# fperezgamonal/flownet2-tf

Hardware: AMD Instinct MI355X
Metric: forward pairs/sec at 512x384 (FlowNet2) (higher is better)
Workload: dtype f16x2 (split fp16 hi+lo operands, 3 fp16 MFMAs per product, fp32 accumulate); 1 GPU; FlowNet2 forward, batch=4 synthetic 512x384 pairs per GPU, seeded synthetic weights; pairs_per_gpu=4, parallelism=dp1 (no collective)

## Files before the change

### flownet2-tf_amd/csrc/conv.hip

```cpp
#include "conv_common.h"
#include <cstdlib>

namespace fn2 {

template <typename T, typename OutT, int TC, int WC, int WP>
__global__ void __launch_bounds__(256) conv_igemm_kernel(const ConvArgs p) {
  constexpr int CH = 16 / (int)sizeof(T);
  constexpr int BC = WC * TC * 16;
  constexpr int BP = WP * 64;
  constexpr int NT = 256;
  static_assert(WC * WP == 4, "4 waves per block");
  constexpr int NPR = BP / 64;
  constexpr int NWR = (BC * 4 + NT - 1) / NT;
  constexpr int WSWZ_BIT = (TC == 4) ? 5 : (TC == 2) ? 4 : 3;
  __shared__ uint4 lds[2][(BC + BP) * 4];

  const int tid = threadIdx.x, lane = tid & 63, wave = tid >> 6;
  const int wc = wave / WP, wp = wave % WP;
  const int cid = tid & 3;

  int pad_y = p.pad, pad_x = p.pad, oy_off = 0, ox_off = 0, osc = 1;
  const T* wgt = reinterpret_cast<const T*>(p.wgt);
  const int phase = blockIdx.z / p.splitk, split = blockIdx.z - phase * p.splitk;
  if (p.deconv) {
// ... 528 lines not shown
      if (oy >= 0 && oy < H && ox >= 0 && ox < W) {
        const bool inner = ey >= E && ey < E + TY && ex >= E && ex < E + TX;
        float2* po = reinterpret_cast<float2*>(pf + (((long)n * H + oy) * W + ox) * 2);
        if (ring && (oy == 0 || oy == H - 1 || ox == 0 || ox == W - 1)) {
          const float2 v = *po;
          a0 = v.x; a1 = v.y;
        } else {
          a0 = b0; a1 = b1;
#pragma unroll
          for (int ky = 0; ky < NT; ++ky)
#pragma unroll
            for (int kx = 0; kx < NT; ++kx) {
              const float2 v = sm[((ey + ky) * RW + ex + kx) * NTAP + ky * NT + kx];
              a0 += v.x; a1 += v.y;
            }
          if (inner) *po = make_float2(a0, a1);
        }
      }
      spf[e] = make_float2(a0, a1);
    }
    if constexpr (UP) {
      __syncthreads();
      const float ub0 = up_bias ? up_bias[0] : 0.f, ub1 = up_bias ? up_bias[1] : 0.f;
      for (int o = tid; o < 4 * TY * TX; o += 256) {
        const int uy = o / (2 * TX), ux = o - uy * (2 * TX);
        const int oy = 2 * ty * TY + uy, ox = 2 * tx * TX + ux;
        if (oy >= 2 * H || ox >= 2 * W) continue;
        const int a = uy & 1, b = ux & 1, y = uy >> 1, x = ux >> 1;
        float r0 = ub0, r1 = ub1;
#pragma unroll
        for (int tty = 0; tty < 2; ++tty) {
          const int iy = y - 1 + a + tty, ky = 3 - a - 2 * tty;
          const int gy = ty * TY + iy;
          if (gy < 0 || gy >= H) continue;
#pragma unroll
          for (int ttx = 0; ttx < 2; ++ttx) {
            const int ix = x - 1 + b + ttx, kx = 3 - b - 2 * ttx;
            const int gx = tx * TX + ix;
            if (gx < 0 || gx >= W) continue;
            const float2 v = spf[(iy + E) * EW + ix + E];
            const float* ww = sw + (ky * 4 + kx) * 4;
            r0 += v.x * ww[0] + v.y * ww[1];
            r1 += v.x * ww[2] + v.y * ww[3];
          }
        }
        OutT* po = up + (((size_t)n * 2 * H + oy) * 2 * W + ox) * up_cs + up_c0;
        if constexpr (is_x2<OutT>::value) {
          const size_t addr = reinterpret_cast<size_t>(po);
          _Float16* g = reinterpret_cast<_Float16*>(addr & ~size_t(31));
          const int j = (int)((addr & 31) >> 2);
          typedef __attribute__((ext_vector_type(2))) _Float16 h2;
          const _Float16 h0 = (_Float16)r0, h1 = (_Float16)r1;
          *reinterpret_cast<h2*>(g + j) = h2{h0, h1};
          *reinterpret_cast<h2*>(g + 8 + j) = h2{(_Float16)(r0 - (float)h0), (_Float16)(r1 - (float)h1)};
        } else {
          store_elem<OutT>(po, r0);
          store_elem<OutT>(po + 1, r1);
        }
      }
    }
    __syncthreads();
  }
}

__global__ void __launch_bounds__(256) head_ring_kernel(const x2_t* __restrict__ in, int in_cs, int in_c0, int cin_groups,
                                                        const float* __restrict__ wc, const float* __restrict__ bc,
                                                        float* __restrict__ pf, int N, int H, int W) {
  const int lane = threadIdx.x & 63;
  const long wave = ((long)blockIdx.x * blockDim.x + threadIdx.x) >> 6;
  const long nwaves = ((long)gridDim.x * blockDim.x) >> 6;
  const int ring = 2 * W + 2 * (H - 2);
  const int nitems = 25 * cin_groups;
  const size_t case_stride = (size_t)nitems * 8 * 2;
  for (long m = wave; m < (long)N * ring; m += nwaves) {
    const int n = (int)(m / ring), r = (int)(m - (long)n * ring);
    int y, x;
    if (r < W) { y = 0; x = r; }
    else if (r < 2 * W) { y = H - 1; x = r - W; }
    else { const int q = r - 2 * W; y = 1 + (q >> 1); x = (q & 1) ? W - 1 : 0; }
    const int cy = y == 0 ? 0 : (y == H - 1 ? 2 : 1), cx = x == 0 ? 0 : (x == W - 1 ? 2 : 1);
    const int cs = 3 * cy + cx;
    const float* w = wc + (size_t)cs * case_stride;
// ... 672 lines not shown
  a.h5_tiles = (int)blocks;
  long total = blocks;
  if (ring && ring_w != nullptr) {
    FN2_REQUIRE(ring_b != nullptr, "flow_head5: ring_w without ring_b");
    a.h5_wc = ring_w; a.h5_bc = ring_b; a.h5_groups = (x->c + 7) / 8;
    FN2_REQUIRE(x->c0 + a.h5_groups * 8 <= x->cs, "flow_head5: the last 8-channel group reaches past the buffer");
    total += cdiv((long)x->n * (2 * x->w + 2 * (x->h - 2)), 16);
  }
  {
    const char* e = getenv("FN2_H5_STRIP");
    if ((a.ksteps == 3 || a.ksteps == 6) && !(e && atoi(e) == 0) && !(a.dbg & 10)) {
      const int nstrip = cdiv(x->w, 60);
      const char* eb = getenv("FN2_H5_BLOCKS");
      const int target = eb ? atoi(eb) : 256;
      const int segs = std::max(1, std::min(x->h, target / std::max(1, x->n * nstrip)));
      const int rows = cdiv(x->h, segs);
      a.h5_tx = nstrip; a.h5_ty = cdiv(x->h, rows); a.h5_rows = rows;
      return launch_head5_strip(a, x->n * a.h5_ty * a.h5_tx, (hipStream_t)stream);
    }
  }
  return launch_head5(a, (int)total, (hipStream_t)stream);
}

int fn2_flow_head_ring(const fn2_tensor* x, const float* wc, const float* bc, float* pf, void* stream) {
  int rc = check_view(x, "flow_head_ring input");
  if (rc) return rc;
  FN2_REQUIRE(wc && bc && pf, "flow_head_ring: null pointer");
  FN2_REQUIRE(x->dtype == FN2_F16X2 && x->cs % 8 == 0 && x->c0 % 8 == 0, "flow_head_ring: split-fp16 input, 8-aligned view");
  FN2_REQUIRE(x->h >= 3 && x->w >= 3, "flow_head_ring: h, w >= 3");
  const int groups = (x->c + 7) / 8;
  FN2_REQUIRE(x->c0 + groups * 8 <= x->cs, "flow_head_ring: the last 8-channel group reaches past the buffer");
  const long ring = (long)x->n * (2 * x->w + 2 * (x->h - 2));
  hipLaunchKernelGGL(head_ring_kernel, dim3(grid_for(ring * 64, 256)), dim3(256), 0, (hipStream_t)stream, (const x2_t*)x->data,
                     x->cs, x->c0, groups, wc, bc, pf, x->n, x->h, x->w);
  FN2_CHECK_LAUNCH("flow_head_ring");
  return FN2_OK;
}

int fn2_upsample_flow(const float* in, const float* w, const float* bias, const fn2_tensor* out, int n, int h, int wd,
                      void* stream) {
  FN2_REQUIRE(in && w, "upsample_flow: null pointer");
  int rc = check_view(out, "upsample_flow output");
  if (rc) return rc;
  FN2_REQUIRE(out->c == 2 && out->n == n && out->h == 2 * h && out->w == 2 * wd,
              "upsample_flow: output view must be [n, 2h, 2w, 2]");
  const long total = (long)n * 4 * h * wd;
// ... 58 lines not shown
```

### flownet2-tf_amd/csrc/conv2.hip

```cpp
#include "conv_common.h"

#include <type_traits>
#include <algorithm>
#include <utility>

#ifndef FN2_X2_ORDER
#define FN2_X2_ORDER 0
#endif
#ifndef FN2_CONV_ABLATE
#define FN2_CONV_ABLATE 0
#endif
#ifndef FN2_SETPRIO
#define FN2_SETPRIO 1
#endif

namespace fn2 {

typedef __attribute__((address_space(3))) void* lptr_t;

constexpr unsigned kOobOffset = 0x80000000u;

typedef int v4i_t __attribute__((ext_vector_type(4)));
typedef unsigned u32x4_t __attribute__((ext_vector_type(4)));

// ... 65 lines not shown
    a1 += __shfl_xor(a1, off, 64);
  }
  if (lane == 0)
    *reinterpret_cast<float2*>(pf + (((size_t)n * H + y) * W + x) * 2) = make_float2(a0 + p.h5_bc[2 * cs], a1 + p.h5_bc[2 * cs + 1]);
}

__device__ __forceinline__ void h5_ring_block(const ConvArgs& p, int rb) {
  const int wave = threadIdx.x >> 6;
  const long total = (long)p.N * (2 * p.OW + 2 * (p.OH - 2));
  for (int k = 0; k < 4; ++k) {
    const long m = (long)rb * 16 + wave * 4 + k;
    if (m >= total) return;
    h5_ring_pixel(p, m);
  }
}

__device__ __forceinline__ float* h5_t(uint4* a, uint4* b, int half, int w) {
  const int byte = w * 4;
  return byte < half ? reinterpret_cast<float*>(reinterpret_cast<char*>(a) + byte)
                     : reinterpret_cast<float*>(reinterpret_cast<char*>(b) + (byte - half));
}

template <typename T, typename OutT, int WC, int WP, int TCN = 2, int TPN = 2, int STAGES = 2, int KG = 1, bool M16 = false,
          bool WREG = false, bool SLAB = false, bool HEAD5 = false, bool FEED = false>
__global__ void __launch_bounds__(256 * KG + (FEED ? 256 : 0)) conv_igemm2_kernel(const ConvArgs p) {
#if defined(__HIP_DEVICE_COMPILE__)
  constexpr int CH = 16 / (int)sizeof(T);
  constexpr int ESZ = (int)sizeof(T);
  constexpr int BC = WC * TCN * 32, BP = WP * TPN * 32;
  static_assert(WC * WP == 4, "4 waves per block");
  constexpr int NWI = BC / 32;
  constexpr int NPI = BP / 32;
  static_assert(!WREG || (is_x2<T>::value && TCN == 1 && KG == 1 && (STAGES == 2 || STAGES == 3) && !M16),
                "WREG: split fp16, one cout tile per wave, two-stage loop or 3-slot ring");
  constexpr int BOFF = WREG ? 0 : BC;
  constexpr int kWTileBytes = (32 * TPN * (TCN * 32 + 4) + 32 * TPN) * 4;
  constexpr int kPoolHalfRows = (STAGES * BP * 128 / 2 > 2 * kWTileBytes ? STAGES * BP * 128 / 2 : 2 * kWTileBytes) / 128 + 1;
  constexpr int ROWS = WREG ? kPoolHalfRows : BC + BP;
  static_assert(KG == 1 || STAGES == 2, "K groups run the two-stage loop");
  constexpr bool kDeep = STAGES > 3;
  __shared__ uint4 lds0_all[(kDeep ? STAGES : WREG ? 2 : KG) * ROWS * 8];
  __shared__ uint4 lds1_all[(kDeep || WREG) ? 1 : KG * ROWS * 8];
  __shared__ uint4 lds2_own[(STAGES == 3 && !WREG) ? ROWS * 8 : 1];

  if constexpr (HEAD5) {
    if ((int)blockIdx.x >= p.h5_tiles) {
      h5_ring_block(p, (int)blockIdx.x - p.h5_tiles);
      return;
    }
  }
  if constexpr (WREG && SLAB && is_x2<T>::value) {
    if (p.fh_M > 0 && (int)blockIdx.z >= p.fh_z0) {
      if (FEED && threadIdx.x >= 256) return;
      float* part = reinterpret_cast<float*>(lds0_all);
      const long e = (((long)blockIdx.z - p.fh_z0) * gridDim.y + blockIdx.y) * gridDim.x + blockIdx.x;
      const long total = (long)(gridDim.z - p.fh_z0) * gridDim.y * gridDim.x;
      for (long m = e; m < p.fh_M; m += total)
        fh_pixel(reinterpret_cast<const x2_t*>(p.in), p.H, p.W, p.in_cs, p.in_c0, p.fh_groups, p.fh_w, p.fh_w + p.fh_w1,
                 p.fh_bias, p.fh_scale, p.fh_out + (size_t)m * p.fh_out_cs + p.fh_out_c0, m, part);
      return;
    }
  }
  const int tid = threadIdx.x, lane = tid & 63;
  const int wave_all = __builtin_amdgcn_readfirstlane(tid >> 6);
  const int grp = KG > 1 ? wave_all >> 2 : 0;
  static_assert(!FEED || (WREG && STAGES == 3 && KG == 1), "FEED: the WREG ring");
  const bool feeder = FEED && wave_all >= 4;
  const int wave = (KG > 1 || FEED) ? wave_all & 3 : wave_all;
  uint4* const lds0 = lds0_all + grp * (ROWS * 8);
  uint4* const lds1 = WREG ? lds0_all + BP * 8 : kDeep ? lds0_all + ROWS * 8 : lds1_all + grp * (ROWS * 8);
  uint4* const lds2 = WREG ? lds0_all + 2 * BP * 8 : lds2_own;
  uint4* const ep1 = (kDeep || WREG) ? lds0_all + ROWS * 8 : lds1_all;
  const int wc = wave / WP, wp = wave % WP;

  int pad_y = p.pad, pad_x = p.pad, oy_off = 0, ox_off = 0, osc = 1;
  const T* wgt = reinterpret_cast<const T*>(p.wgt);
  const int phase = blockIdx.z / p.splitk, split = blockIdx.z - phase * p.splitk;
  const unsigned wrow_bytes = (unsigned)p.ksteps * 128u;
  if (p.deconv) {
    const int a = phase >> 1, b = phase & 1;
    pad_y = a ? p.ph_pad1 : p.ph_pad0; pad_x = b ? p.ph_pad1 : p.ph_pad0; oy_off = a; ox_off = b; osc = 2;
    wgt += (size_t)phase * p.cout_pad * (wrow_bytes / ESZ);
  }
  const int khi = p.deconv ? p.kh_ph[phase >> 1] : p.KH, kwi = p.deconv ? p.kw_ph[phase & 1] : p.KW;
  const int nst_all = (p.cin_chunks >> 3) * khi * kwi;
  const int kt0 = split * p.kper + grp;
  const int kt1 = (FN2_CONV_ABLATE && (p.dbg & 1048576)) ? kt0 : min(nst_all, split * p.kper + p.kper);
  int bx = blockIdx.x, by = blockIdx.y;
  if (!(p.dbg & 4)) {
    const int NT = HEAD5 ? p.h5_tiles : gridDim.x * gridDim.y, L = blockIdx.x + gridDim.x * blockIdx.y;
    const int xcd = L & 7, chunk = NT >> 3, rem = NT & 7;
    const int Lp = xcd * chunk + min(xcd, rem) + (L >> 3);
    if (p.wmajor) {
      by = Lp / (int)gridDim.x;
      bx = Lp - by * (int)gridDim.x;
    } else {
      bx = Lp / (int)gridDim.y;
      by = Lp - bx * (int)gridDim.y;
    }
  }
  const int m0 = bx * BP;
  const int c0 = by * BC;

  const v4i_t rsrc_w = make_rsrc(wgt, (int)(p.cout_pad * wrow_bytes));
  const v4i_t rsrc_x = make_rsrc(p.in, p.in_bytes);

  const int lrow = lane >> 3, lphys = lane & 7;
  unsigned woff[NWI];
#pragma unroll
  for (int j = 0; j < NWI; ++j) {
    const int row = wave * (BC / 4) + j * 8 + lrow;
    woff[j] = (unsigned)(c0 + row) * wrow_bytes + (unsigned)((lphys ^ ((row >> 1) & 7)) * 16);
  }
  int roff[NPI];
  unsigned vmask[NPI];
#pragma unroll
  for (int j = 0; j < NPI; ++j) {
    const int row = wave * (BP / 4) + j * 8 + lrow;
    const int m = m0 + row;
    bool v = m < p.M;
    const int mm = v ? m : 0;
    int n = mm / (p.OH * p.OW);
    const int rem = mm - n * (p.OH * p.OW);
    int oy = rem / p.OW, ox = rem - oy * p.OW;
    if constexpr (HEAD5) {
      static_assert(BP == 256, "HEAD5: 8 x 32 positions per block");
      const int tx = bx % p.h5_tx, tyn = bx / p.h5_tx;
      n = tyn / p.h5_ty;
      oy = (tyn - n * p.h5_ty) * 4 - 2 + (row >> 5);
      ox = tx * 28 - 2 + (row & 31);
      v = true;
    }
    const int iy0 = oy * p.stride - pad_y, ix0 = ox * p.stride - pad_x;
    roff[j] = (((n * p.H + iy0) * p.W + ix0) * p.in_cs + p.in_c0) * ESZ + (lphys ^ ((row >> 1) & 7)) * 16;
    unsigned mk = 0;
    if (v) {
      for (int k = 0; k < p.KH; ++k) mk |= (unsigned)(iy0 + k >= 0 && iy0 + k < p.H) << k;
      for (int k = 0; k < p.KW; ++k) mk |= (unsigned)(ix0 + k >= 0 && ix0 + k < p.W) << (8 + k);
    }
    vmask[j] = mk;
  }
  const int spt = p.cin_chunks >> 3;
  const int ntap = khi * kwi;
  const bool tap_outer = FN2_CONV_ABLATE && (p.dbg & 16);
  int sc = tap_outer ? kt0 % spt : kt0 / ntap;
  int tap = tap_outer ? kt0 / spt : kt0 - sc * ntap;
  int ky = tap / kwi, kx = tap - ky * kwi;
  int wstage = kt0;

  auto issue_piece = [&](auto piece_c, uint4* lds) {
    constexpr int i = decltype(piece_c)::value;
    if constexpr (i < NWI) {
      if constexpr (!WREG) {
// ... 356 lines not shown
            *reinterpret_cast<float4*>(h5_t(lds0_all, lds1_all, ROWS * 128, pos * TS + cb + 4 * q)) =
                make_float4(acc[tc][tp][4 * q] * p.out_scale, acc[tc][tp][4 * q + 1] * p.out_scale,
                            acc[tc][tp][4 * q + 2] * p.out_scale, acc[tc][tp][4 * q + 3] * p.out_scale);
      }
    __syncthreads();
    if (p.dbg & 8) return;
    const int tx = bx % p.h5_tx, tyn = bx / p.h5_tx;
    const int n = tyn / p.h5_ty, ty = tyn - n * p.h5_ty;
    float* pf = reinterpret_cast<float*>(p.out);
    if (tid < 224) {
      const int o = tid & 1, px = tid >> 1;
      const int py = px / 28, pxx = px - py * 28;
      const int oy = ty * 4 + py, ox = tx * 28 + pxx;
      if (oy < p.OH && ox < p.OW && !(p.h5_ring && (oy == 0 || oy == p.OH - 1 || ox == 0 || ox == p.OW - 1))) {
        float a = p.bias ? p.bias[o] : 0.f;
#pragma unroll
        for (int uy = 0; uy < 5; ++uy)
#pragma unroll
          for (int ux = 0; ux < 5; ++ux)
            a += *h5_t(lds0_all, lds1_all, ROWS * 128, ((py + uy) * 32 + pxx + ux) * TS + (uy * 5 + ux) * 2 + o);
        pf[(((size_t)n * p.OH + oy) * p.OW + ox) * 2 + o] = a;
      }
    }
    return;
  }
  if (FN2_CONV_ABLATE && (p.dbg & 262144)) return;
  if constexpr (M16) {
    OutT* out16 = reinterpret_cast<OutT*>(p.out);
    const int r16 = lane & 15, g16 = lane >> 4;
    float* slab = p.splitk > 1 ? p.ws + (size_t)split * p.N * p.out_H * p.out_W * p.ws_cs : nullptr;
#pragma unroll
    for (int b = 0; b < TPN * 2; ++b) {
      const int m = m0 + wp * TPN * 32 + b * 16 + r16;
      if (m >= p.M) continue;
      const int n = m / (p.OH * p.OW);
      const int rem = m - n * (p.OH * p.OW);
      const int oy = rem / p.OW, ox = rem - oy * p.OW;
      const size_t opix = ((size_t)n * p.out_H + (oy * osc + oy_off)) * p.out_W + (ox * osc + ox_off);
      OutT* po = out16 + opix * p.out_cs + p.out_c0;
#pragma unroll
      for (int a = 0; a < TCN * 2; ++a) {
        const int co = c0 + wc * TCN * 32 + (a >> 1) * 32 + 16 * (g16 & 1) + 8 * (a & 1) + 4 * (g16 >> 1);
        if (slab != nullptr) {
          if (co < p.ws_cs)
            *reinterpret_cast<float4*>(slab + opix * p.ws_cs + co) =
                make_float4(acc16[a][b][0], acc16[a][b][1], acc16[a][b][2], acc16[a][b][3]);
// ... 915 lines not shown
  else if (tile == 128 && a.bp64 && a.kg == 2) FN2_LAUNCH2(cdiv(a.M, 64), a.cout_pad / 128, 512, 2, 2, 2, 1, 2, 2);
  else if (tile == 128 && a.bp64 == 3) FN2_LAUNCH2(cdiv(a.M, 64), a.cout_pad / 128, 256, 2, 2, 2, 1, 6, 1);
  else if (tile == 128 && a.bp64 == 2) FN2_LAUNCH2(cdiv(a.M, 64), a.cout_pad / 128, 256, 2, 2, 2, 1, 3, 1);
  else if (tile == 128 && a.bp64) FN2_LAUNCH2(cdiv(a.M, 64), a.cout_pad / 128, 256, 2, 2, 2, 1, 2, 1);
  else if (tile == 128) FN2_LAUNCH2(cdiv(a.M, 128), a.cout_pad / 128, 256, 2, 2, 2, 2, 2, 1);
  else if (tile == 64 && a.bp64) FN2_LAUNCH2(cdiv(a.M, 128), a.cout_pad / 64, 256, 1, 4, 2, 1, 2, 1);
  else if (tile == 64) FN2_LAUNCH2(cdiv(a.M, 256), a.cout_pad / 64, 256, 1, 4, 2, 2, 2, 1);
  else if (a.bp64) FN2_LAUNCH2(cdiv(a.M, 128), a.cout_pad / 32, 256, 1, 4, 1, 1, 2, 1);
  else FN2_LAUNCH2(cdiv(a.M, 256), a.cout_pad / 32, 256, 1, 4, 1, 2, 2, 1);
#undef FN2_LAUNCH2
  FN2_CHECK_LAUNCH("conv_igemm2");
  return FN2_OK;
}

int launch_head5_strip(const ConvArgs& a, int blocks, hipStream_t s) {
  if (a.ksteps == 3) hipLaunchKernelGGL((head5_strip_kernel<1>), dim3(blocks), dim3(512), 0, s, a);
  else if (a.ksteps == 6) hipLaunchKernelGGL((head5_strip_kernel<2>), dim3(blocks), dim3(512), 0, s, a);
  else return fail(FN2_ERR_UNSUPPORTED, "flow_head5 strip form: %d channel lines (3 or 6)", a.ksteps);
  FN2_CHECK_LAUNCH("flow_head5_strip");
  return FN2_OK;
}

int launch_head5(const ConvArgs& a, int blocks, hipStream_t s) {
  hipLaunchKernelGGL((conv_igemm2_kernel<x2_t, float, 1, 4, 2, 2, 2, 1, false, false, false, true>), dim3(blocks, 1, 1), dim3(256), 0,
                     s, a);
  FN2_CHECK_LAUNCH("flow_head5");
  return FN2_OK;
}

bool conv_fast_ok(int in_dtype, int cin_pad, int cout) {
  const int esz = dtype_size(in_dtype);
  return cout > 2 && (cin_pad * esz) % 128 == 0;
}

int launch_conv_fast(const ConvArgs& a, int in_dtype, int out_dtype, int tile, int phases, hipStream_t s) {
  if (tile != 128 && tile != 64 && tile != 32) return fail(FN2_ERR_UNSUPPORTED, "conv fast path: cout tile %d", tile);
  if (in_dtype == FN2_F32) return launch2<float, float>(a, tile, phases, s);
  if (in_dtype == FN2_BF16) {
    if (out_dtype == FN2_BF16) return launch2<bf16_t, bf16_t>(a, tile, phases, s);
    return launch2<bf16_t, float>(a, tile, phases, s);
  }
  if (in_dtype == FN2_F16) {
    if (out_dtype == FN2_F16) return launch2<f16_t, f16_t>(a, tile, phases, s);
    return launch2<f16_t, float>(a, tile, phases, s);
  }
  if (out_dtype == FN2_F16X2) {
    if (launch_rowrun<x2_t>(a, tile, phases, s)) { FN2_CHECK_LAUNCH("conv_rowrun"); return FN2_OK; }
    if (launch_stem<x2_t>(a, tile, phases, s)) { FN2_CHECK_LAUNCH("conv_stem"); return FN2_OK; }
    if (launch_halo<x2_t>(a, tile, phases, s)) { FN2_CHECK_LAUNCH("conv_halo"); return FN2_OK; }
// ... 10 lines not shown
```

### flownet2-tf_amd/csrc/conv_common.h

```cpp
#pragma once
#include "fn2_common.h"

namespace fn2 {

struct ConvArgs {
  const void* in;
  const void* wgt;
  const float* bias;
  void* out;
  int N, H, W, in_cs, in_c0;
  int cin_chunks;
  int KH, KW, stride, pad;
  int OH, OW;
  int M;
  int out_H, out_W, out_cs, out_c0, Cout;
  int ksteps;
  int cout_pad;
  int act;
  int deconv;
  int ph_pad0, ph_pad1;
  int kh_ph[2], kw_ph[2];
  int merged;
  int wmajor;
  int bp64;
  int KH_KW_hint;
  int kg;
  int h5_tx, h5_ty, h5_ring;
  int h5_tiles, h5_groups;
  const float* h5_wc;
  const float* h5_bc;
  int h5_rows;
  int fh_M, fh_z0;
  const float* fh_w;
  int fh_w1, fh_groups;
  const float* fh_bias;
  float* fh_out;
  int fh_out_cs, fh_out_c0;
  float fh_scale;
  const float* up_src; const float* up_w; const float* up_bias; int up_c0;
  int wfrag;
  int accum;
  int vec_ok;
  int splitk;
  int kper;
  float* ws;
  int ws_cs;
  float out_scale;
  int in_bytes;
  const void* mask_y;
  int mask_c0, mask_c1;
  int dbg;
};

__device__ __forceinline__ void fh_pixel(const x2_t* __restrict__ in, int H, int W, int in_cs, int in_c0, int groups,
// ... 56 lines not shown
        load16<OutT>(po, o);
#pragma unroll
        for (int q = 0; q < 16; ++q) v[q] += o[q];
      }
      if (mask) {
        float y[16];
        load16<OutT>(reinterpret_cast<const OutT*>(p.mask_y) + (po - out_base), y);
#pragma unroll
        for (int q = 0; q < 16; ++q)
          if (cout_base + q >= p.mask_c0 && cout_base + q < p.mask_c1) v[q] *= y[q] > 0.f ? 1.f : (y[q] < 0.f ? 0.1f : 0.55f);
      }
    } else {
#pragma unroll
      for (int q = 0; q < 16; ++q)
        if (cout_base + q < p.Cout) {
          if (p.accum) v[q] += load_elem<OutT>(po + q);
          v[q] = act_grad<OutT>(p, out_base, po + q, cout_base + q, v[q]);
        }
    }
  }
}

template <typename OutT>
__device__ __forceinline__ void store4(OutT* p, float a, float b, float c, float d) {
  const float v[4] = {a, b, c, d};
  store_vec<OutT, 4>(p, v);
}

struct ConvNameSink { char* buf; int cap; };
ConvNameSink& conv_name_sink();

int launch_conv_fast(const ConvArgs& a, int in_dtype, int out_dtype, int tile, int phases, hipStream_t s);
int launch_head5(const ConvArgs& a, int blocks, hipStream_t s);
int launch_head5_strip(const ConvArgs& a, int blocks, hipStream_t s);
bool conv_fast_ok(int in_dtype, int cin_pad, int cout);

}
```

### flownet2-tf_amd/src/_hip.py

```python
import ctypes as C
import os

import numpy as np
import torch

_HERE = os.path.dirname(os.path.abspath(__file__))
LIB_PATH = os.path.join(os.path.dirname(_HERE), "lib", "libflownet2_hip.so")

FN2_F32, FN2_BF16, FN2_F16, FN2_F16X2 = 0, 1, 2, 3
ACT_NONE, ACT_LEAKY = 0, 1
OK = 0
ERR_INVALID_ARGUMENT, ERR_UNSUPPORTED, ERR_HIP = -1, -2, -3


class Fn2Tensor(C.Structure):
    _fields_ = [("data", C.c_void_p), ("dtype", C.c_int32), ("n", C.c_int32), ("h", C.c_int32),
                ("w", C.c_int32), ("c", C.c_int32), ("cs", C.c_int32), ("c0", C.c_int32)]


class Fn2ConvPlan(C.Structure):
    _fields_ = [("layout", C.c_int32), ("cout_tile", C.c_int32), ("kstep_elems", C.c_int32),
                ("wgt_dtype", C.c_int32)]


# ... 28 lines not shown
    "fn2_correlation_f32_ws": (_i, [_p, _p, _p] + [_i] * 9 + [_p, C.c_int64, _p]),
    "fn2_correlation_grad_f32": (_i, [_p] * 5 + [_i] * 9 + [_p]),
    "fn2_flow_warp_f32": (_i, [_p, _p, _p, _i, _i, _i, _i, _p]),
    "fn2_flow_warp_grad_f32": (_i, [_p] * 5 + [_i] * 4 + [_p]),
    "fn2_downsample_f32": (_i, [_p, _p] + [_i] * 6 + [_p]),
    "fn2_downsample_scaled_f32": (_i, [_p, _f, _p] + [_i] * 6 + [_p]),
    "fn2_fill_zero": (_i, [_p, C.c_int64, _p]),
    "fn2_add_f32": (_i, [_p, _p, C.c_int64, _p]),
    "fn2_slice_copy_f32": (_i, [_tp, _p, _p]),
    "fn2_resize_bilinear_f32": (_i, [_p, _p] + [_i] * 6 + [_f, _p]),
    "fn2_conv2d_plan": (_i, [_i, _i, _i, C.POINTER(Fn2ConvPlan)]),
    "fn2_conv2d_workspace_bytes": (C.c_int64, [C.POINTER(Fn2ConvDesc)]),
    "fn2_conv2d": (_i, [C.POINTER(Fn2ConvDesc), _p]),
    "fn2_conv2d_kernel_name": (_i, [C.POINTER(Fn2ConvDesc), C.c_char_p, _i]),
    "fn2_conv2d_splits": (_i, [C.POINTER(Fn2ConvDesc)]),
    "fn2_augment_f32": (_i, [_p, _p, _p, _p, _i, _i, _i, _i, _i, _i, _p]),
    "fn2_flow_augmentation_f32": (_i, [_p, _p, _p, _p, _i, _i, _i, _i, _i, _p]),
    "fn2_flow_head_gather": (_i, [_p, _i, _p, _p, _i, _i, _i, _p]),
    "fn2_upsample_flow": (_i, [_p, _p, _p, _tp, _i, _i, _i, _p]),
    "fn2_flow_head_tail": (_i, [_p, _i, _i, _p, _p, _i, _i, _i, _i, _p, _p, _tp, _p]),
    "fn2_flow_head_tail_slabs": (_i, [_p, _i, _i, C.c_int64, _f, _i, _p, _p, _i, _i, _i, _i, _p, _p, _tp, _p]),
    "fn2_flow_head_ring": (_i, [_tp, _p, _p, _p, _p]),
    "fn2_flow_head5": (_i, [_tp, _p, _i, _i, _f, _p, _p, _i, _p, _p, _p]),
    "fn2_u8_to_f32_lut": (_i, [_p, _p, _p, C.c_int64, _p]),
    "fn2_pack_pair": (_i, [_p, _p, _tp, _i, _p]),
    "fn2_pack_interp_u8": (_i, [_p, _p, _p, _p, _p, _tp, _i, _p]),
    "fn2_pack_image": (_i, [_p, _i, _tp, _i, _i, _p]),
    "fn2_pack_image_s2d": (_i, [_p, _i, _i, _i, _tp, _i, _i, _p]),
    "fn2_correlation_fused": (_i, [_tp, _tp, _tp, _i, _i, _i, _p]),
    "fn2_stack_input": (_i, [_p, _p, _p, _tp, _i, _p]),
    "fn2_fusion_input": (_i, [_p, _p, _p, _p, _tp, _i, _p]),
    "fn2_stack_input_pf": (_i, [_p, _p, _p, _i, _i, _f, _p, _tp, _i, _p]),
    "fn2_fusion_input_pf": (_i, [_p, _p, _p, _f, _p, _p, _f, _p, _i, _i, _tp, _i, _p]),
    "fn2_epe_loss_grad": (_i, [_p, _p, _p, _p, _i, _i, _i, _f, _f, _p]),
    "fn2_epe_loss_grad_weighted": (_i, [_p, _p, _p, _p, _p, _i, _i, _i, _f, _f, _p]),
    "fn2_leaky_bwd": (_i, [_tp, _tp, _p, _p]),
    "fn2_bias_grad": (_i, [_tp, _p, _p]),
    "fn2_gather_f32": (_i, [_p, _p, _p, C.c_int64, _p]),
    "fn2_to_f16x2": (_i, [_p, _p, _p, C.c_int64, _f, _p]),
    "fn2_to_f16x2_frag": (_i, [_p, _p, _p, C.c_int64, _f, _i, _p]),
    "fn2_adam_step": (_i, [_p, _p, _p, _p, C.c_int64, _f, _f, _f, _f, _i, _f, _f, _p]),
    "fn2_adam_step_multi": (_i, [_p, _p, _p, _i, _f, _f, _f, _f, _i, _f, _p]),
    "fn2_adam_step_multi_dev": (_i, [_p, _p, _p, _i, _p, _p]),
    "fn2_upsample_flow_bwd": (_i, [_tp, _p, _p, _p, _p, _i, _p]),
    "fn2_head_bwd_filter": (_i, [_tp, _p, _p, _i, _i, _p]),
    "fn2_head_g18": (_i, [_p, _tp, _p]),
# ... 99 lines not shown
```

### flownet2-tf_amd/src/engine.py

```python
import ctypes as C
import math
import os

import numpy as np
import torch

from . import _hip, netdefs, weights as W

_DT = {"f32": torch.float32, "bf16": torch.bfloat16, "f16": torch.float16, "f16x2": torch.float32}
_CODE = {"f32": _hip.FN2_F32, "bf16": _hip.FN2_BF16, "f16": _hip.FN2_F16, "f16x2": _hip.FN2_F16X2}
_TILE_ARGS = {128: "2, 2, 2, 2", 64: "1, 4, 2, 2", 32: "1, 4, 1, 2"}


def conv2_kernel_args(tile, m, cout_pad, phases, x2=True):
    dbg = int(os.environ.get("FN2_CONV_DBG", "0"))
    blocks64 = -(-m // 64) * (cout_pad // 128) * phases if tile == 128 else 0
    big = "FN2_M16_MIN" in os.environ and blocks64 >= max(int(os.environ["FN2_M16_MIN"]), 513)
    m16 = "true" if (x2 and not dbg & 512 and (dbg & 1024 or big)) else "false"
    full = dbg & 32
    if tile < 128:
        base = {64: "1, 4, 2, 2, 2, 1", 32: "1, 4, 1, 2, 2, 1"}[tile] if full else {64: "1, 4, 2, 1, 2, 1", 32: "1, 4, 1, 1, 2, 1"}[tile]
        return f"{base}, {m16}"
    blocks = -(-m // 64) * (cout_pad // 128) * phases
    if not full and int(os.environ.get("FN2_KG", "1")):
# ... 314 lines not shown
    def _head_gemm(self, scope, spec, src, dst, up=None):
        name, kind, k, stride, pad, cin, cout, act = spec
        sbuf, sc0, sc = src
        pf = dst[0]
        in_code = self._code(sbuf)
        esz = 2 if in_code in (_hip.FN2_BF16, _hip.FN2_F16) else 4
        cin_line = _round_up(cin, 128 // esz)
        if sc0 + cin_line > sbuf.shape[3]:
            return False
        plan = _hip.conv_plan(in_code, cin_line, 18)
        if plan.layout != 1:
            return False
        w = np.asarray(self._w(f"{scope}/{name}/weights"), np.float32)
        w1 = np.ascontiguousarray(w.transpose(2, 0, 1, 3)).reshape(1, 1, cin, 18)
        packed, cin_pad, cout_pad, kpad = W.pack_conv(w1, plan.cout_tile, plan.kstep_elems, cin_line, plan.layout)
        out_scale = 1.0
        if plan.wgt_dtype == _hip.FN2_F16X2:
            wmax = float(abs(packed).max())
            if wmax > 0:
                k2 = int(math.floor(math.log2(1024.0 / wmax)))
                packed, out_scale = packed * (2.0 ** k2), 2.0 ** (-k2)
        wdev = W.packed_to_device(packed, plan.wgt_dtype, self.device)
        bias = self._bias(scope, name, kind, cout)
        if self._head_t is None:
            self._head_t = {}
        if self._branch not in self._head_t:
            self._head_t[self._branch] = torch.zeros((self.N * self.H * self.W, 32), dtype=torch.float32, device=self.device)
        head_t = self._head_t[self._branch]
        n, h, wd = pf.shape[0], pf.shape[1], pf.shape[2]
        d = _hip.Fn2ConvDesc()
        d.inp = self._v(sbuf, sc, sc0)
        d.out = _hip.Fn2Tensor(head_t.data_ptr(), _hip.FN2_F32, n, h, wd, 18, 32, 0)
        d.wgt, d.bias = wdev.data_ptr(), None
        d.kind, d.kh, d.kw, d.stride, d.pad = 0, 1, 1, 1, 0
        d.act = _hip.ACT_NONE
        d.cin_pad, d.cout_pad, d.kpad, d.wgt_layout = cin_pad, cout_pad, kpad, plan.layout
        d.out_scale = out_scale
        self.keep += [d, wdev, bias]
        self.conv_descs.append(d)
        self.desc_branch.append(self._branch)
        tn = _TNAME[self.dtype_name] if in_code == self.act_code else "float"
        self._op(f"{scope}/{name}", self.lib.fn2_conv2d, C.byref(d),
                 kernel=f"conv_igemm2_kernel<{tn}, float, {conv2_kernel_args(plan.cout_tile, 0, cout_pad, 1, tn == 'fn2::x2_t')}>")
        t_ptr, t_cs, nslab, slab, tscale = self._head_slabs(d, head_t, 32)
        if up is not None and int(os.environ.get("FN2_FUSE_UPFLOW", "1")):
            up_name, (ubuf, uc0, uc) = up
            uw = W.to_device(self._w(f"{scope}/{up_name}/weights"), torch.float32, self.device)
            ub = self._bias(scope, up_name, "deconv", 2)
            uv = self._v(ubuf, uc, uc0)
            self.keep += [uw, ub, uv]
            self.layers.append(dict(scope=scope, name=up_name, kind="upflow", src=pf, dst=up[1], w=uw, b=ub, view=uv))
            self._op(f"{scope}/{name}/tail+{up_name}", self.lib.fn2_flow_head_tail_slabs, t_ptr, t_cs, nslab, slab,
# ... 28 lines not shown
        wc = np.zeros((9, 25, groups * 8, 2), np.float32)
        wc[:, :, :sc, :] = w5.reshape(9, 25, sc, 2)
        wcd = W.to_device(wc, torch.float32, self.device)
        bcd = W.to_device(bias5.astype(np.float32), torch.float32, self.device)
        vin = self._v(sbuf, sc, sc0)
        self.keep += [wcd, bcd, vin]
        w1x1 = np.ascontiguousarray(w5[4].transpose(2, 0, 1, 3)).reshape(1, 1, sc, 50).astype(np.float32)
        packed, cin_pad, cout_pad, kpad = W.pack_conv(w1x1, plan.cout_tile, plan.kstep_elems, cin_line, plan.layout)
        out_scale = 1.0
        wmax = float(abs(packed).max())
        if wmax > 0:
            k2 = int(math.floor(math.log2(1024.0 / wmax)))
            packed, out_scale = packed * (2.0 ** k2), 2.0 ** (-k2)
        wdev = W.packed_to_device(packed, plan.wgt_dtype, self.device)
        cm = ic_spec[6]
        if n * h * wd >= int(os.environ.get("FN2_HEAD5_MIN", "65536")) and plan.cout_tile == 64 and kpad == cin_pad:
            b5 = W.to_device(bias5[4].astype(np.float32), torch.float32, self.device)
            vx = self._v(sbuf, sc, sc0)
            self.keep += [wdev, b5, vx]
            strip = cin_pad in (96, 192) and int(os.environ.get("FN2_H5_STRIP", "1"))
            self._op(f"{scope}/{ic_name}+{pf_name}", self.lib.fn2_flow_head5, C.byref(vx), _hip.ptr(wdev), cin_pad, kpad,
                     C.c_float(out_scale), _hip.ptr(b5), _hip.ptr(pf), 1, _hip.ptr(wcd), _hip.ptr(bcd),
                     kernel=("head5_strip_kernel<%d>" % (cin_pad // 96)) if strip else
                     "conv_igemm2_kernel<fn2::x2_t, float, 1, 4, 2, 2, 2, 1, false, false, false, true>")
            self.layer_flops.append((f"{scope}/{ic_name}+{pf_name}", 2.0 * n * h * wd * 9 * (sc * cm + cm * 2)))
            self.layer_io_bytes.append((f"{scope}/{ic_name}+{pf_name}", float(n * h * wd * (sc * 4 + 2 * 4) + 9 * (sc * cm + 2 * cm) * 4)))
            return 1
        self._op(f"{scope}/{pf_name}/ring", self.lib.fn2_flow_head_ring, C.byref(vin), _hip.ptr(wcd), _hip.ptr(bcd), _hip.ptr(pf),
                 kernel="flow_head_ring")
        if self._head_t is None:
            self._head_t = {}
        key = (self._branch, 64)
        if key not in self._head_t:
            self._head_t[key] = torch.zeros((self.N * self.H * self.W, 64), dtype=torch.float32, device=self.device)
        head_t = self._head_t[key]
        d = _hip.Fn2ConvDesc()
        d.inp = self._v(sbuf, sc, sc0)
        d.out = _hip.Fn2Tensor(head_t.data_ptr(), _hip.FN2_F32, n, h, wd, 50, 64, 0)
        d.wgt, d.bias = wdev.data_ptr(), None
        d.kind, d.kh, d.kw, d.stride, d.pad = 0, 1, 1, 1, 0
        d.act = _hip.ACT_NONE
        d.cin_pad, d.cout_pad, d.kpad, d.wgt_layout = cin_pad, cout_pad, kpad, plan.layout
        d.out_scale = out_scale
        b5 = W.to_device(bias5[4].astype(np.float32), torch.float32, self.device)
        self.keep += [d, wdev, b5]
        self.conv_descs.append(d)
        self.desc_branch.append(self._branch)
# ... 587 lines not shown
```

### include/flownet2_hip.h

```cpp
#ifndef FLOWNET2_HIP_H_
#define FLOWNET2_HIP_H_

#include <stddef.h>
#include <stdint.h>

#ifdef __cplusplus
extern "C" {
#endif

typedef enum {
  FN2_OK = 0,
  FN2_ERR_INVALID_ARGUMENT = -1,
  FN2_ERR_UNSUPPORTED = -2,
  FN2_ERR_HIP = -3
} fn2_status;

typedef enum { FN2_F32 = 0, FN2_BF16 = 1, FN2_F16 = 2, FN2_F16X2 = 3 } fn2_dtype;

typedef enum { FN2_ACT_NONE = 0, FN2_ACT_LEAKY = 1  } fn2_act;

typedef struct {
  void* data;
  int32_t dtype;
  int32_t n, h, w;
// ... 64 lines not shown
  const float* up_bias;
  int32_t up_c0;
  const void* head;
  int32_t raw_partials;
} fn2_conv_desc;

typedef struct {
  int32_t layout, cout_tile, kstep_elems, wgt_dtype;
} fn2_conv_plan;
int fn2_conv2d_plan(int in_dtype, int cin_pad, int cout, fn2_conv_plan* plan);
int64_t fn2_conv2d_workspace_bytes(const fn2_conv_desc* d);
int fn2_conv2d(const fn2_conv_desc* d, void* stream);
int fn2_conv2d_kernel_name(const fn2_conv_desc* desc, char* name, int cap);
int fn2_conv2d_splits(const fn2_conv_desc* desc);

int fn2_flow_head_gather(const float* t, int t_cs, const float* bias, float* out, int n, int h, int w, void* stream);
int fn2_flow_head_tail(const float* t, int t_cs, int taps, const float* bias, float* pf, int n, int h, int w, int ring,
                       const float* up_w, const float* up_bias, const fn2_tensor* up_out, void* stream);
int fn2_flow_head_tail_slabs(const float* t, int t_cs, int nslab, int64_t slab_stride, float scale, int taps, const float* bias,
                             float* pf, int n, int h, int w, int ring, const float* up_w, const float* up_bias,
                             const fn2_tensor* up_out, void* stream);
int fn2_flow_head5(const fn2_tensor* x, const void* wgt, int cin_pad, int kpad, float out_scale, const float* bias, float* pf,
                   int ring, const float* ring_w, const float* ring_b, void* stream);
int fn2_flow_head_ring(const fn2_tensor* x, const float* wc, const float* bc, float* pf, void* stream);
int fn2_upsample_flow(const float* in, const float* w, const float* bias, const fn2_tensor* out, int n, int h, int wd,
                      void* stream);

int fn2_u8_to_f32_lut(const unsigned char* src, const float* lut256, float* dst, long count, void* stream);

int fn2_pack_pair(const float* a, const float* b, const fn2_tensor* out, int pad, void* stream);
int fn2_pack_interp_u8(const unsigned char* img, const unsigned char* mask, const float* sparse, const float* lut256,
                       const unsigned char* flags, const fn2_tensor* out, int pad, void* stream);
int fn2_pack_image(const float* img, int n_img, const fn2_tensor* out, int n0, int pad, void* stream);
int fn2_pack_image_s2d(const float* img, int n_img, int h, int w, const fn2_tensor* out, int n0, int pad, void* stream);

int fn2_correlation_fused(const fn2_tensor* a, const fn2_tensor* b, const fn2_tensor* out,
                          int max_displacement, int stride_2, int act, void* stream);

int fn2_stack_input(const float* a, const float* b, const float* flow, const fn2_tensor* out, int pad,
                    void* stream);

int fn2_fusion_input(const float* a, const float* b, const float* flow_sd, const float* flow_css,
                     const fn2_tensor* out, int pad, void* stream);
int fn2_stack_input_pf(const float* a, const float* b, const float* pf, int pf_h, int pf_w, float scale, float* flow_out,
                       const fn2_tensor* out, int pad, void* stream);
int fn2_fusion_input_pf(const float* a, const float* b, const float* pf_sd, float scale_sd, float* flow_sd_out,
// ... 59 lines not shown
```

Before: 1134 pairs/s.

## Fuse 3x3 flow head conv, tap gather and flow upsample into one kernel

```diff
diff --git a/flownet2-tf_amd/csrc/conv.hip b/flownet2-tf_amd/csrc/conv.hip
--- a/flownet2-tf_amd/csrc/conv.hip
+++ b/flownet2-tf_amd/csrc/conv.hip
@@ -574,42 +574,7 @@
     if constexpr (UP) {
       __syncthreads();
       const float ub0 = up_bias ? up_bias[0] : 0.f, ub1 = up_bias ? up_bias[1] : 0.f;
-      for (int o = tid; o < 4 * TY * TX; o += 256) {
-        const int uy = o / (2 * TX), ux = o - uy * (2 * TX);
-        const int oy = 2 * ty * TY + uy, ox = 2 * tx * TX + ux;
-        if (oy >= 2 * H || ox >= 2 * W) continue;
-        const int a = uy & 1, b = ux & 1, y = uy >> 1, x = ux >> 1;
-        float r0 = ub0, r1 = ub1;
-#pragma unroll
-        for (int tty = 0; tty < 2; ++tty) {
-          const int iy = y - 1 + a + tty, ky = 3 - a - 2 * tty;
-          const int gy = ty * TY + iy;
-          if (gy < 0 || gy >= H) continue;
-#pragma unroll
-          for (int ttx = 0; ttx < 2; ++ttx) {
-            const int ix = x - 1 + b + ttx, kx = 3 - b - 2 * ttx;
-            const int gx = tx * TX + ix;
-            if (gx < 0 || gx >= W) continue;
-            const float2 v = spf[(iy + E) * EW + ix + E];
-            const float* ww = sw + (ky * 4 + kx) * 4;
-            r0 += v.x * ww[0] + v.y * ww[1];
-            r1 += v.x * ww[2] + v.y * ww[3];
-          }
-        }
-        OutT* po = up + (((size_t)n * 2 * H + oy) * 2 * W + ox) * up_cs + up_c0;
-        if constexpr (is_x2<OutT>::value) {
-          const size_t addr = reinterpret_cast<size_t>(po);
-          _Float16* g = reinterpret_cast<_Float16*>(addr & ~size_t(31));
-          const int j = (int)((addr & 31) >> 2);
-          typedef __attribute__((ext_vector_type(2))) _Float16 h2;
-          const _Float16 h0 = (_Float16)r0, h1 = (_Float16)r1;
-          *reinterpret_cast<h2*>(g + j) = h2{h0, h1};
-          *reinterpret_cast<h2*>(g + 8 + j) = h2{(_Float16)(r0 - (float)h0), (_Float16)(r1 - (float)h1)};
-        } else {
-          store_elem<OutT>(po, r0);
-          store_elem<OutT>(po + 1, r1);
-        }
-      }
+      upsample_flow_tile<OutT>(spf, sw, ub0, ub1, n, ty * TY, tx * TX, TY, TX, H, W, up, up_cs, up_c0);
     }
     __syncthreads();
   }
@@ -1328,6 +1293,51 @@
   return launch_head5(a, (int)total, (hipStream_t)stream);
 }
 
+int fn2_flow_head3(const fn2_tensor* x, const void* wgt, int cin_pad, int kpad, float out_scale, const float* bias, float* pf,
+                   const float* up_w, const float* up_bias, const fn2_tensor* up_out, void* stream) {
+  int rc = check_view(x, "flow_head3 input");
+  if (rc) return rc;
+  FN2_REQUIRE(wgt && pf, "flow_head3: null pointer");
+  FN2_REQUIRE(x->dtype == FN2_F16X2 && x->cs % 8 == 0 && x->c0 % 8 == 0, "flow_head3: split-fp16 input, 8-aligned view");
+  FN2_REQUIRE(cin_pad % 32 == 0 && cin_pad >= x->c && x->c0 + cin_pad <= x->cs && kpad == cin_pad,
+              "flow_head3: the channel run must be whole 128-byte lines inside the buffer (kpad = cin_pad)");
+  const long in_bytes = (long)x->n * x->h * x->w * x->cs * 4;
+  FN2_REQUIRE(in_bytes < (1L << 31), "flow_head3: input buffer >= 2 GiB is not addressable by the LDS-DMA kernel");
+  const bool up = up_w != nullptr;
+  if (up) {
+    rc = check_view(up_out, "flow_head3 upsample output");
+    if (rc) return rc;
+    FN2_REQUIRE(up_out->c == 2 && up_out->n == x->n && up_out->h == 2 * x->h && up_out->w == 2 * x->w,
+                "flow_head3: the upsample view must be [n, 2h, 2w, 2]");
+    if (up_out->dtype == FN2_F16X2) FN2_REQUIRE(up_out->c0 % 2 == 0, "flow_head3: split-fp16 slice must start at an even channel");
+  }
+  ConvArgs a = {};
+  a.in = x->data; a.wgt = wgt; a.bias = bias; a.out = pf;
+  a.N = x->n; a.H = x->h; a.W = x->w; a.in_cs = x->cs; a.in_c0 = x->c0;
+  a.cin_chunks = cin_pad / 4;
+  a.KH = a.KW = 1; a.stride = 1; a.pad = 0;
+  a.OH = x->h; a.OW = x->w;
+  a.h3_halo = up ? 2 : 1;
+  a.h5_tx = cdiv(x->w, 32 - 2 * a.h3_halo); a.h5_ty = cdiv(x->h, 8 - 2 * a.h3_halo);
+  const long blocks = (long)x->n * a.h5_ty * a.h5_tx;
+  FN2_REQUIRE(blocks * 256 < (1L << 31), "flow_head3: too many tiles");
+  a.M = (int)(blocks * 256);
+  a.h5_tiles = (int)blocks;
+  a.out_H = x->h; a.out_W = x->w; a.out_cs = 2; a.out_c0 = 0; a.Cout = 2;
+  a.ksteps = cin_pad / 32;
+  a.cout_pad = 32;
+  a.act = FN2_ACT_NONE;
+  a.kh_ph[0] = a.kh_ph[1] = a.kw_ph[0] = a.kw_ph[1] = 1;
+  a.kg = 1; a.splitk = 1; a.kper = a.ksteps; a.ws = nullptr; a.ws_cs = 4;
+  a.out_scale = out_scale == 0.f ? 1.f : out_scale;
+  a.in_bytes = (int)in_bytes;
+  if (up) {
+    a.up_w = up_w; a.up_bias = up_bias; a.up_c0 = up_out->c0;
+    a.h3_up = up_out->data; a.h3_up_cs = up_out->cs;
+  }
+  return launch_head3(a, (int)blocks, up ? up_out->dtype : FN2_F32, (hipStream_t)stream);
+}
+
 int fn2_flow_head_ring(const fn2_tensor* x, const float* wc, const float* bc, float* pf, void* stream) {
   int rc = check_view(x, "flow_head_ring input");
   if (rc) return rc;
diff --git a/flownet2-tf_amd/csrc/conv2.hip b/flownet2-tf_amd/csrc/conv2.hip
--- a/flownet2-tf_amd/csrc/conv2.hip
+++ b/flownet2-tf_amd/csrc/conv2.hip
@@ -111,7 +111,7 @@
 }
 
 template <typename T, typename OutT, int WC, int WP, int TCN = 2, int TPN = 2, int STAGES = 2, int KG = 1, bool M16 = false,
-          bool WREG = false, bool SLAB = false, bool HEAD5 = false, bool FEED = false>
+          bool WREG = false, bool SLAB = false, int HEAD = 0, bool FEED = false>
 __global__ void __launch_bounds__(256 * KG + (FEED ? 256 : 0)) conv_igemm2_kernel(const ConvArgs p) {
 #if defined(__HIP_DEVICE_COMPILE__)
   constexpr int CH = 16 / (int)sizeof(T);
@@ -132,6 +132,8 @@
   __shared__ uint4 lds1_all[(kDeep || WREG) ? 1 : KG * ROWS * 8];
   __shared__ uint4 lds2_own[(STAGES == 3 && !WREG) ? ROWS * 8 : 1];
 
+  static_assert(HEAD == 0 || HEAD == 3 || HEAD == 5, "HEAD: 0 (a convolution), 3 or 5 (flow heads)");
+  constexpr bool HEAD5 = HEAD == 5;
   if constexpr (HEAD5) {
     if ((int)blockIdx.x >= p.h5_tiles) {
       h5_ring_block(p, (int)blockIdx.x - p.h5_tiles);
@@ -177,7 +179,7 @@
   const int kt1 = (FN2_CONV_ABLATE && (p.dbg & 1048576)) ? kt0 : min(nst_all, split * p.kper + p.kper);
   int bx = blockIdx.x, by = blockIdx.y;
   if (!(p.dbg & 4)) {
-    const int NT = HEAD5 ? p.h5_tiles : gridDim.x * gridDim.y, L = blockIdx.x + gridDim.x * blockIdx.y;
+    const int NT = HEAD ? p.h5_tiles : gridDim.x * gridDim.y, L = blockIdx.x + gridDim.x * blockIdx.y;
     const int xcd = L & 7, chunk = NT >> 3, rem = NT & 7;
     const int Lp = xcd * chunk + min(xcd, rem) + (L >> 3);
     if (p.wmajor) {
@@ -212,12 +214,13 @@
     int n = mm / (p.OH * p.OW);
     const int rem = mm - n * (p.OH * p.OW);
     int oy = rem / p.OW, ox = rem - oy * p.OW;
-    if constexpr (HEAD5) {
-      static_assert(BP == 256, "HEAD5: 8 x 32 positions per block");
+    if constexpr (HEAD != 0) {
+      static_assert(BP == 256, "HEAD: 8 x 32 positions per block");
+      const int halo = HEAD5 ? 2 : p.h3_halo;
       const int tx = bx % p.h5_tx, tyn = bx / p.h5_tx;
       n = tyn / p.h5_ty;
-      oy = (tyn - n * p.h5_ty) * 4 - 2 + (row >> 5);
-      ox = tx * 28 - 2 + (row & 31);
+      oy = (tyn - n * p.h5_ty) * (8 - 2 * halo) - halo + (row >> 5);
+      ox = tx * (32 - 2 * halo) - halo + (row & 31);
       v = true;
     }
     const int iy0 = oy * p.stride - pad_y, ix0 = ox * p.stride - pad_x;
@@ -620,6 +623,54 @@
         pf[(((size_t)n * p.OH + oy) * p.OW + ox) * 2 + o] = a;
       }
     }
+    return;
+  }
+  if constexpr (HEAD == 3) {
+    static_assert(TCN == 1 && STAGES == 2 && KG == 1 && !WREG && !M16, "HEAD 3: one 32-row cout tile, two-stage loop");
+    constexpr int TS = 20, EH = 6, EW = 30;
+    static_assert((256 * TS + EH * EW * 2 + 64) * 4 <= ROWS * 128, "the table, the flow tile and the upsample weights fit a stage buffer");
+    float* const tab = reinterpret_cast<float*>(lds0_all);
+    float2* const spf = reinterpret_cast<float2*>(tab + 256 * TS);
+    float* const sw = tab + 256 * TS + EH * EW * 2;
+    const bool up = p.h3_up != nullptr;
+#pragma unroll
+    for (int tp = 0; tp < TPN; ++tp) {
+      const int pos = wp * TPN * 32 + tp * 32 + fr;
+#pragma unroll
+      for (int q = 0; q < 4; ++q)
+        if (fh * 16 + 4 * q < TS)
+          *reinterpret_cast<float4*>(tab + pos * TS + fh * 16 + 4 * q) =
+              make_float4(acc[0][tp][4 * q] * p.out_scale, acc[0][tp][4 * q + 1] * p.out_scale,
+                          acc[0][tp][4 * q + 2] * p.out_scale, acc[0][tp][4 * q + 3] * p.out_scale);
+    }
+    if (up && tid < 64) sw[tid] = p.up_w[tid];
+    __syncthreads();
+    const int halo = p.h3_halo, TY = 8 - 2 * halo, TX = 32 - 2 * halo, E = halo - 1;
+    const int tx = bx % p.h5_tx, tyn = bx / p.h5_tx;
+    const int n = tyn / p.h5_ty, ty = tyn - n * p.h5_ty;
+    float* pf = reinterpret_cast<float*>(p.out);
+    if (tid < EH * EW) {
+      const int ey = tid / EW, ex = tid - ey * EW;
+      const int oy = ty * TY - E + ey, ox = tx * TX - E + ex;
+      float a0 = 0.f, a1 = 0.f;
+      if (oy >= 0 && oy < p.OH && ox >= 0 && ox < p.OW) {
+        a0 = p.bias ? p.bias[0] : 0.f; a1 = p.bias ? p.bias[1] : 0.f;
+#pragma unroll
+        for (int ky = 0; ky < 3; ++ky)
+#pragma unroll
+          for (int kx = 0; kx < 3; ++kx) {
+            const float2 v = *reinterpret_cast<const float2*>(tab + ((ey + ky) * 32 + ex + kx) * TS + (ky * 3 + kx) * 2);
+            a0 += v.x; a1 += v.y;
+          }
+        if (ey >= E && ey < E + TY && ex >= E && ex < E + TX)
+          *reinterpret_cast<float2*>(pf + (((size_t)n * p.OH + oy) * p.OW + ox) * 2) = make_float2(a0, a1);
+      }
+      spf[tid] = make_float2(a0, a1);
+    }
+    if (!up) return;
+    __syncthreads();
+    upsample_flow_tile<OutT>(spf, sw, p.up_bias ? p.up_bias[0] : 0.f, p.up_bias ? p.up_bias[1] : 0.f, n, ty * TY, tx * TX, TY, TX,
+                             p.OH, p.OW, reinterpret_cast<OutT*>(p.h3_up), p.h3_up_cs, p.up_c0);
     return;
   }
   if (FN2_CONV_ABLATE && (p.dbg & 262144)) return;
@@ -1581,9 +1632,27 @@
 }
 
 int launch_head5(const ConvArgs& a, int blocks, hipStream_t s) {
-  hipLaunchKernelGGL((conv_igemm2_kernel<x2_t, float, 1, 4, 2, 2, 2, 1, false, false, false, true>), dim3(blocks, 1, 1), dim3(256), 0,
+  hipLaunchKernelGGL((conv_igemm2_kernel<x2_t, float, 1, 4, 2, 2, 2, 1, false, false, false, 5>), dim3(blocks, 1, 1), dim3(256), 0,
                      s, a);
   FN2_CHECK_LAUNCH("flow_head5");
+  return FN2_OK;
+}
+
+template <typename UpT>
+static void launch_head3_t(const ConvArgs& a, int blocks, hipStream_t s) {
+  if (conv_name_sink().buf)
+    snprintf(conv_name_sink().buf, conv_name_sink().cap, "conv_igemm2_kernel<fn2::x2_t, %s, 1, 4, 1, 2, 2, 1, false, false, false, 3>",
+             type_name<UpT>());
+  else
+    hipLaunchKernelGGL((conv_igemm2_kernel<x2_t, UpT, 1, 4, 1, 2, 2, 1, false, false, false, 3>), dim3(blocks, 1, 1), dim3(256), 0, s, a);
+}
+
+int launch_head3(const ConvArgs& a, int blocks, int up_dtype, hipStream_t s) {
+  if (a.h3_up == nullptr || up_dtype == FN2_F32) launch_head3_t<float>(a, blocks, s);
+  else if (up_dtype == FN2_F16X2) launch_head3_t<x2_t>(a, blocks, s);
+  else if (up_dtype == FN2_BF16) launch_head3_t<bf16_t>(a, blocks, s);
+  else launch_head3_t<f16_t>(a, blocks, s);
+  FN2_CHECK_LAUNCH("flow_head3");
   return FN2_OK;
 }
 
diff --git a/flownet2-tf_amd/csrc/conv_common.h b/flownet2-tf_amd/csrc/conv_common.h
--- a/flownet2-tf_amd/csrc/conv_common.h
+++ b/flownet2-tf_amd/csrc/conv_common.h
@@ -30,6 +30,9 @@
   const float* h5_wc;
   const float* h5_bc;
   int h5_rows;
+  int h3_halo;
+  void* h3_up;
+  int h3_up_cs;
   int fh_M, fh_z0;
   const float* fh_w;
   int fh_w1, fh_groups;
@@ -132,6 +135,49 @@
 }
 
 template <typename OutT>
+__device__ __forceinline__ void upsample_flow_tile(const float2* __restrict__ spf, const float* __restrict__ sw, float ub0,
+                                                   float ub1, int n, int y0, int x0, int TY, int TX, int H, int W,
+                                                   OutT* __restrict__ up, int up_cs, int up_c0) {
+  const int EW = TX + 2;
+  for (int o = threadIdx.x; o < 4 * TY * TX; o += 256) {
+    const int uy = o / (2 * TX), ux = o - uy * (2 * TX);
+    const int oy = 2 * y0 + uy, ox = 2 * x0 + ux;
+    if (oy >= 2 * H || ox >= 2 * W) continue;
+    const int a = uy & 1, b = ux & 1, y = uy >> 1, x = ux >> 1;
+    float r0 = ub0, r1 = ub1;
+#pragma unroll
+    for (int tty = 0; tty < 2; ++tty) {
+      const int iy = y - 1 + a + tty, ky = 3 - a - 2 * tty;
+      const int gy = y0 + iy;
+      if (gy < 0 || gy >= H) continue;
+#pragma unroll
+      for (int ttx = 0; ttx < 2; ++ttx) {
+        const int ix = x - 1 + b + ttx, kx = 3 - b - 2 * ttx;
+        const int gx = x0 + ix;
+        if (gx < 0 || gx >= W) continue;
+        const float2 v = spf[(iy + 1) * EW + ix + 1];
+        const float* ww = sw + (ky * 4 + kx) * 4;
+        r0 += v.x * ww[0] + v.y * ww[1];
+        r1 += v.x * ww[2] + v.y * ww[3];
+      }
+    }
+    OutT* po = up + (((size_t)n * 2 * H + oy) * 2 * W + ox) * up_cs + up_c0;
+    if constexpr (is_x2<OutT>::value) {
+      const size_t addr = reinterpret_cast<size_t>(po);
+      _Float16* g = reinterpret_cast<_Float16*>(addr & ~size_t(31));
+      const int j = (int)((addr & 31) >> 2);
+      typedef __attribute__((ext_vector_type(2))) _Float16 h2;
+      const _Float16 h0 = (_Float16)r0, h1 = (_Float16)r1;
+      *reinterpret_cast<h2*>(g + j) = h2{h0, h1};
+      *reinterpret_cast<h2*>(g + 8 + j) = h2{(_Float16)(r0 - (float)h0), (_Float16)(r1 - (float)h1)};
+    } else {
+      store_elem<OutT>(po, r0);
+      store_elem<OutT>(po + 1, r1);
+    }
+  }
+}
+
+template <typename OutT>
 __device__ __forceinline__ void store4(OutT* p, float a, float b, float c, float d) {
   const float v[4] = {a, b, c, d};
   store_vec<OutT, 4>(p, v);
@@ -143,6 +189,7 @@
 int launch_conv_fast(const ConvArgs& a, int in_dtype, int out_dtype, int tile, int phases, hipStream_t s);
 int launch_head5(const ConvArgs& a, int blocks, hipStream_t s);
 int launch_head5_strip(const ConvArgs& a, int blocks, hipStream_t s);
+int launch_head3(const ConvArgs& a, int blocks, int up_dtype, hipStream_t s);
 bool conv_fast_ok(int in_dtype, int cin_pad, int cout);
 
 }
diff --git a/flownet2-tf_amd/src/_hip.py b/flownet2-tf_amd/src/_hip.py
--- a/flownet2-tf_amd/src/_hip.py
+++ b/flownet2-tf_amd/src/_hip.py
@@ -74,6 +74,7 @@
     "fn2_flow_head_tail_slabs": (_i, [_p, _i, _i, C.c_int64, _f, _i, _p, _p, _i, _i, _i, _i, _p, _p, _tp, _p]),
     "fn2_flow_head_ring": (_i, [_tp, _p, _p, _p, _p]),
     "fn2_flow_head5": (_i, [_tp, _p, _i, _i, _f, _p, _p, _i, _p, _p, _p]),
+    "fn2_flow_head3": (_i, [_tp, _p, _i, _i, _f, _p, _p, _p, _p, _tp, _p]),
     "fn2_u8_to_f32_lut": (_i, [_p, _p, _p, C.c_int64, _p]),
     "fn2_pack_pair": (_i, [_p, _p, _tp, _i, _p]),
     "fn2_pack_interp_u8": (_i, [_p, _p, _p, _p, _p, _tp, _i, _p]),
diff --git a/flownet2-tf_amd/src/engine.py b/flownet2-tf_amd/src/engine.py
--- a/flownet2-tf_amd/src/engine.py
+++ b/flownet2-tf_amd/src/engine.py
@@ -360,12 +360,34 @@
                 packed, out_scale = packed * (2.0 ** k2), 2.0 ** (-k2)
         wdev = W.packed_to_device(packed, plan.wgt_dtype, self.device)
         bias = self._bias(scope, name, kind, cout)
+        n, h, wd = pf.shape[0], pf.shape[1], pf.shape[2]
+        if (n * h * wd >= int(os.environ.get("FN2_HEAD3_MIN", "8192")) and in_code == _hip.FN2_F16X2 and plan.cout_tile == 32
+                and kpad == cin_pad and sc0 % 8 == 0 and sbuf.shape[3] % 8 == 0 and sbuf.numel() * 4 < 2 ** 31):
+            vx = self._v(sbuf, sc, sc0)
+            self.keep += [wdev, bias, vx]
+            fuse = up is not None and bool(int(os.environ.get("FN2_FUSE_UPFLOW", "1")))
+            uw = ub = uv = None
+            if fuse:
+                up_name, (ubuf, uc0, uc) = up
+                uw = W.to_device(self._w(f"{scope}/{up_name}/weights"), torch.float32, self.device)
+                ub = self._bias(scope, up_name, "deconv", 2)
+                uv = self._v(ubuf, uc, uc0)
+                self.keep += [uw, ub, uv]
+                self.layers.append(dict(scope=scope, name=up_name, kind="upflow", src=pf, dst=up[1], w=uw, b=ub, view=uv))
+            on = {_hip.FN2_F32: "float", _hip.FN2_F16X2: "fn2::x2_t", _hip.FN2_BF16: "__bf16", _hip.FN2_F16: "_Float16"}[
+                self._code(up[1][0]) if fuse else _hip.FN2_F32]
+            self._op(f"{scope}/{name}", self.lib.fn2_flow_head3, C.byref(vx), _hip.ptr(wdev), cin_pad,
+                     kpad, C.c_float(out_scale), _hip.ptr(bias) if bias is not None else None, _hip.ptr(pf),
+                     _hip.ptr(uw) if fuse else None, _hip.ptr(ub) if ub is not None else None, C.byref(uv) if fuse else None,
+                     kernel=f"conv_igemm2_kernel<fn2::x2_t, {on}, 1, 4, 1, 2, 2, 1, false, false, false, 3>")
+            self.layer_flops.append((f"{scope}/{name}", 2.0 * n * h * wd * 9 * cin * 2))
+            self.layer_io_bytes.append((f"{scope}/{name}", float(n * h * wd * (cin * esz + 2 * 4) + 18 * cin * esz)))
+            return True
         if self._head_t is None:
             self._head_t = {}
         if self._branch not in self._head_t:
             self._head_t[self._branch] = torch.zeros((self.N * self.H * self.W, 32), dtype=torch.float32, device=self.device)
         head_t = self._head_t[self._branch]
-        n, h, wd = pf.shape[0], pf.shape[1], pf.shape[2]
         d = _hip.Fn2ConvDesc()
         d.inp = self._v(sbuf, sc, sc0)
         d.out = _hip.Fn2Tensor(head_t.data_ptr(), _hip.FN2_F32, n, h, wd, 18, 32, 0)
@@ -440,7 +462,7 @@
             self._op(f"{scope}/{ic_name}+{pf_name}", self.lib.fn2_flow_head5, C.byref(vx), _hip.ptr(wdev), cin_pad, kpad,
                      C.c_float(out_scale), _hip.ptr(b5), _hip.ptr(pf), 1, _hip.ptr(wcd), _hip.ptr(bcd),
                      kernel=("head5_strip_kernel<%d>" % (cin_pad // 96)) if strip else
-                     "conv_igemm2_kernel<fn2::x2_t, float, 1, 4, 2, 2, 2, 1, false, false, false, true>")
+                     "conv_igemm2_kernel<fn2::x2_t, float, 1, 4, 2, 2, 2, 1, false, false, false, 5>")
             self.layer_flops.append((f"{scope}/{ic_name}+{pf_name}", 2.0 * n * h * wd * 9 * (sc * cm + cm * 2)))
             self.layer_io_bytes.append((f"{scope}/{ic_name}+{pf_name}", float(n * h * wd * (sc * 4 + 2 * 4) + 9 * (sc * cm + 2 * cm) * 4)))
             return 1
diff --git a/include/flownet2_hip.h b/include/flownet2_hip.h
--- a/include/flownet2_hip.h
+++ b/include/flownet2_hip.h
@@ -110,6 +110,8 @@
                              const fn2_tensor* up_out, void* stream);
 int fn2_flow_head5(const fn2_tensor* x, const void* wgt, int cin_pad, int kpad, float out_scale, const float* bias, float* pf,
                    int ring, const float* ring_w, const float* ring_b, void* stream);
+int fn2_flow_head3(const fn2_tensor* x, const void* wgt, int cin_pad, int kpad, float out_scale, const float* bias, float* pf,
+                   const float* up_w, const float* up_bias, const fn2_tensor* up_out, void* stream);
 int fn2_flow_head_ring(const fn2_tensor* x, const float* wc, const float* bc, float* pf, void* stream);
 int fn2_upsample_flow(const float* in, const float* w, const float* bias, const fn2_tensor* out, int n, int h, int wd,
                       void* stream);
```

After: 1144 pairs/s, median of 6. Within noise of the previous version (+0.9%).
